# Immortalqx/pi-slam-fusion

Measured on AMD Instinct MI355X. Metric: keyframes/sec fused (4000x3000 -> 256^2 tiles, 5-band), higher is better.
Workload: dtype f32; 1 GPU; cfg-2/cfg-A: 4000x3000 BGR8 keyframes, serpentine sortie, Map2D.Scale=1, 5-band Laplacian, CV_32FC3 (ForceFloat=1) pyramids, frames resident in HBM; frames_per_rank=2646, sortie_frames_before_timing=20, lookahead=48, rendered_rank0=2666, culled_tiles_rank0=490117

## Files before the change

include/pifusion.h:

```cpp
#ifndef PIFUSION_H
#define PIFUSION_H
#include <stddef.h>
#include <stdint.h>

#ifdef __cplusplus
extern "C" {
#endif

#define PF_ELE_PIXELS 256

enum { PF_TYPE_NONE = 0, PF_TYPE_CPU = 1, PF_TYPE_GPU = 2, PF_TYPE_MULTIBAND = 3, PF_TYPE_RENDER = 4 };

enum { PF_8UC1 = 0, PF_8UC3 = 16, PF_8UC4 = 24, PF_16SC3 = 19, PF_32FC1 = 5, PF_32FC3 = 21 };

typedef struct pf_image {
    int         rows, cols, type;
    const void* data;
    size_t      step;
} pf_image;

typedef struct pf_options {
    int    band_number;
    int    force_float;
    int    high_quality_show;
// ... 109 lines not shown
    unsigned long long strips_sent, strips_received, tiles, peers;
    double plan_ms, pack_ms, exchange_ms, compute_ms;
    unsigned long long verified;
} pf_dist_stats;
int      pf_dist_last_stats(pf_dist* d, pf_dist_stats* out);
typedef struct pf_strip_plan { int peer, ix, iy, dx, dy, tile; unsigned long long offset; } pf_strip_plan;
int      pf_dist_plan_blend(int nranks, int me, const int* counts, const int* lists3, const long long* caps, int high_quality,
                            const size_t halo_bytes9[9], pf_strip_plan* send, int send_cap, int* n_send,
                            pf_strip_plan* recv, int recv_cap, int* n_recv, int* mine_xy, int mine_cap, int* n_mine);
int      pf_dist_info(pf_dist* d, int* rank, int* nranks, const char** transport);
int      pf_dist_set_verify(pf_dist* d, int on);

int     pf_profile_enable(pf_map* m, int mode);
int     pf_profile_read(pf_map* m, int cap, const char** names, double* total_ms, long long* launches,
                        double* alg_bytes);
int     pf_profile_read_run(pf_map* m, int cap, const char** names, double* total_ms, long long* launches,
                            double* alg_bytes, double* alg_bytes_run);
int     pf_profile_reset(pf_map* m);
int     pf_render_stats(pf_map* m, double out4[4]);
int     pf_timer_read(pf_map* m, int cap, const char** names, long long* calls, double* mean_s, double* min_s, double* max_s);
int     pf_timer_reset(pf_map* m);
long long pf_debug_culled_tiles(pf_map* m);
long long pf_debug_culled_cells(pf_map* m);
double  pf_debug_level0_exact_px(pf_map* m);
int     pf_debug_render_log(pf_map* m, long long* out, int cap);
void    pf_set_cull(pf_map* m, int on);
void    pf_debug_form_counts(long long out[8]);
long long pf_debug_compact_launches(void);
int     pf_stats(pf_map* m, long long* rendered, long long* rejected, long long* dropped);
int     pf_reserve_tiles(pf_map* m, long long n_tiles);

#ifdef __cplusplus
}
#endif
#endif
```

pi-slam-fusion_amd/__init__.py:

```python
import ctypes as C
import os
import subprocess

import numpy as np

_HERE = os.path.dirname(os.path.abspath(__file__))
LIB_PATH = os.environ.get("PF_LIB") or os.path.join(_HERE, "libpifusion.so")
ELE_PIXELS = 256

NoType, TypeCPU, TypeGPU, TypeMultiBandCPU, TypeRender = 0, 1, 2, 3, 4
PF_8UC3, PF_8UC4, PF_16SC3, PF_32FC3 = 16, 24, 19, 21


def host_array(shape, dtype=np.uint8):
    n = int(np.prod(shape)) * np.dtype(dtype).itemsize
    p = lib().pf_host_alloc(n)
    if not p:
        raise MemoryError("pf_host_alloc(%d)" % n)
    buf = (C.c_uint8 * n).from_address(p)
    a = np.frombuffer(buf, dtype=dtype).reshape(shape)
    import weakref
    weakref.finalize(buf, lib().pf_host_free, p)
    return a

# ... 116 lines not shown
    L.pf_dist_feed.argtypes = [vp, C.POINTER(Image), dp, C.c_int]
    L.pf_dist_feed_jpeg.argtypes = [vp, C.c_char_p, C.c_size_t, C.c_int, C.c_int, dp, C.c_int]
    L.pf_dist_save.argtypes = [vp, C.c_char_p]
    L.pf_dist_save_to_memory.argtypes = [vp, vp, ip, ip, ip, ip]
    L.pf_dist_last_stats.argtypes = [vp, C.POINTER(DistStats)]
    L.pf_dist_info.argtypes = [vp, ip, ip, C.POINTER(C.c_char_p)]
    L.pf_dist_set_verify.argtypes = [vp, C.c_int]
    L.pf_dist_plan_blend.argtypes = [C.c_int, C.c_int, ip, ip, C.POINTER(C.c_longlong), C.c_int, C.POINTER(C.c_size_t), vp, C.c_int, ip,
                                     vp, C.c_int, ip, ip, C.c_int, ip]
    if hasattr(L, "pf_debug_compact_launches") or not os.environ.get("PF_LIB"):
        L.pf_debug_compact_launches.argtypes = []; L.pf_debug_compact_launches.restype = C.c_longlong
    L.pf_profile_enable.argtypes = [vp, C.c_int]
    L.pf_profile_read.argtypes = [vp, C.c_int, C.POINTER(C.c_char_p), dp, C.POINTER(C.c_longlong), dp]
    if hasattr(L, "pf_profile_read_run") or not os.environ.get("PF_LIB"):
        L.pf_profile_read_run.argtypes = [vp, C.c_int, C.POINTER(C.c_char_p), dp, C.POINTER(C.c_longlong), dp, dp]
    L.pf_profile_reset.argtypes = [vp]
    L.pf_stats.argtypes = [vp, C.POINTER(C.c_longlong), C.POINTER(C.c_longlong), C.POINTER(C.c_longlong)]
    L.pf_reserve_tiles.argtypes = [vp, C.c_longlong]
    L.pf_debug_culled_tiles.argtypes = [vp]; L.pf_debug_culled_tiles.restype = C.c_longlong
    L.pf_set_cull.argtypes = [vp, C.c_int]; L.pf_set_cull.restype = None
    if hasattr(L, "pf_debug_render_log") or not os.environ.get("PF_LIB"):
        L.pf_debug_render_log.argtypes = [vp, C.POINTER(C.c_longlong), C.c_int]
    L.pf_debug_culled_cells.argtypes = [vp]; L.pf_debug_culled_cells.restype = C.c_longlong
    L.pf_debug_level0_exact_px.argtypes = [vp]; L.pf_debug_level0_exact_px.restype = C.c_double
    L.pf_render_stats.argtypes = [vp, dp]
    L.pf_timer_read.argtypes = [vp, C.c_int, C.POINTER(C.c_char_p), C.POINTER(C.c_longlong), dp, dp, dp]
    L.pf_timer_reset.argtypes = [vp]
    _lib = L
    return L


POSE7 = C.c_double * 7


def _pose(p):
    if isinstance(p, POSE7):
        return p, p
    a = np.ascontiguousarray(p, dtype=np.float64).reshape(-1)
    return a, a.ctypes.data_as(C.POINTER(C.c_double))


def default_options(**kw):
    o = Options()
    lib().pf_default_options(C.byref(o))
    for k, v in kw.items():
        if not hasattr(o, k):
# ... 432 lines not shown
        cap = 16
        names = (C.c_char_p * cap)(); calls = (C.c_longlong * cap)(); mean = (C.c_double * cap)(); mn = (C.c_double * cap)(); mx = (C.c_double * cap)()
        k = lib().pf_timer_read(self._h, cap, names, calls, mean, mn, mx)
        return {names[i].decode(): {"calls": calls[i], "mean_s": mean[i], "min_s": mn[i], "max_s": mx[i]} for i in range(k)}

    def timer_reset(self):
        lib().pf_timer_reset(self._h)

    def set_cull(self, on):
        lib().pf_set_cull(self._h, 1 if on else 0)

    def render_log(self):
        n = lib().pf_debug_render_log(self._h, None, 0)
        out = (C.c_longlong * max(n, 1))()
        k = lib().pf_debug_render_log(self._h, out, n)
        return [int(out[i]) for i in range(min(n, k))]

    def culled_tiles(self):
        return int(lib().pf_debug_culled_tiles(self._h))

    def culled_cells(self):
        return int(lib().pf_debug_culled_cells(self._h))

    def stats(self):
        a, b, c = C.c_longlong(), C.c_longlong(), C.c_longlong()
        lib().pf_stats(self._h, C.byref(a), C.byref(b), C.byref(c))
        return {"rendered": a.value, "rejected": b.value, "dropped": c.value}
```

pi-slam-fusion_amd/csrc/c_api.cpp:

```cpp
#include "dist.hpp"
#include "jpeg_device.hpp"
#include <cstdlib>
#include <cmath>
#include <cstdio>
#include <cstring>
#include <algorithm>
#include <vector>
#include <mutex>
#include <new>

using pf::FusionMap;

struct pf_map {
    FusionMap impl;
    pf::JpegDevice jpeg;
    pf_map(int t, bool th, const pf_options& o) : impl(t, th, o) {}
    ~pf_map() { if (impl.ok() && impl.use_device()) impl.sync(); }
};

static std::mutex g_jpeg_mu;
static pf::JpegDevice* shared_jpeg(int device = 0)
{
    static pf::JpegDevice* d[64] = {};
    if (device < 0 || device >= 64) device = 0;
// ... 36 lines not shown
{
    if (type == PF_TYPE_NONE || type == PF_TYPE_RENDER) return nullptr;
    pf_options o;
    if (opt) o = *opt; else pf_default_options(&o);
    pf_map* m = new (std::nothrow) pf_map(type, thread != 0, o);
    if (m && !m->impl.ok()) { delete m; return nullptr; }
    return m;
}

void pf_destroy(pf_map* m) { delete m; }
const char* pf_last_error(void) { return pf::last_error(); }

int pf_prepare(pf_map* m, const double plane[7], const double cam[6], int n, const pf_image* imgs, const double* poses7)
{ return m && m->impl.prepare(plane, cam, n, imgs, poses7); }

int pf_feed(pf_map* m, const pf_image* img, const double pose[7]) { return m && m->impl.feed(img, pose, false); }
int pf_feed_device(pf_map* m, const pf_image* img, const double pose[7]) { return m && m->impl.feed(img, pose, true); }
int pf_debug_phase_stamps(unsigned long long* out, int cap_blocks) { return pf::read_phase_stamps(out, cap_blocks); }
void pf_debug_form_counts(long long out[8]) { if (out) pf::read_form_counts(out); }
long long pf_debug_compact_launches(void) { return pf::read_compact_launches(); }
int pf_debug_render_log(pf_map* m, long long* out, int cap) { return m ? m->impl.render_log(out, cap) : 0; }
void pf_set_cull(pf_map* m, int on) { if (m) m->impl.set_cull(on != 0); }
long long pf_debug_culled_cells(pf_map* m) { return m ? m->impl.culled_cells() : 0; }
double pf_debug_level0_exact_px(pf_map* m) { return m ? m->impl.level0_exact_px() : 0; }
long long pf_debug_culled_tiles(pf_map* m) { return m ? m->impl.culled_tiles() : 0; }
int pf_debug_select_counts(unsigned long long* out, int reset) { return out ? pf::read_select_counts(out, reset) : 0; }
long pf_debug_read_last_frame(pf_map* m, void* out, size_t cap) { return m ? m->impl.read_back_last_frame(out, cap) : -1; }
unsigned pf_queue_size(pf_map* m) { return m ? m->impl.queue_size() : 0; }
int pf_sync(pf_map* m) { return m && m->impl.sync(); }
int pf_save(pf_map* m, const char* filename) { return m && filename && m->impl.save(filename); }
int pf_save_tiff(pf_map* m, const char* filename, int quality, int force_bigtiff) { return m && filename && m->impl.save_tiff(filename, quality, force_bigtiff != 0); }
int pf_save_tiff_masked(pf_map* m, const char* filename, int quality, int force_bigtiff) { return m && filename && m->impl.save_tiff_masked(filename, quality, force_bigtiff != 0); }
int pf_jpeg_info(const uint8_t* data, size_t len, int* rows, int* cols, int* components) { return pf::jpeg_info(data, len, rows, cols, components); }
int pf_jpeg_decode_bgr(const uint8_t* data, size_t len, uint8_t* bgr, int rows, int cols)
{ return rows > 0 && cols > 0 && pf::jpeg_decode_bgr(data, len, bgr, rows, cols, (size_t)cols * 3); }
int pf_jpeg_decode_device(const uint8_t* data, size_t len, void* dev_bgr, int rows, int cols, void* hip_stream)
{
    std::lock_guard<std::mutex> l(g_jpeg_mu);
    if (rows <= 0 || cols <= 0 || !dev_bgr) return 0;
    hipPointerAttribute_t at{};
    if (hipPointerGetAttributes(&at, dev_bgr) != hipSuccess || at.type != hipMemoryTypeDevice) { (void)hipGetLastError(); pf::set_error("pf_jpeg_decode_device: destination is not device memory"); return 0; }
    int prev = 0;
    (void)hipGetDevice(&prev);
    if (at.device != prev && hipSetDevice(at.device) != hipSuccess) { pf::set_error("pf_jpeg_decode_device: hipSetDevice failed"); return 0; }
    const int ok = shared_jpeg(at.device)->decode_to(data, len, (uint8_t*)dev_bgr, rows, cols, hip_stream);
    if (at.device != prev) (void)hipSetDevice(prev);
// ... 341 lines not shown
```

pi-slam-fusion_amd/csrc/frame_plan.hpp:

```cpp
#pragma once
#include "plan_limits.hpp"
#include <algorithm>
#include <cmath>
#include <cstdint>
#include <cstring>
#include <vector>

namespace pf {

struct Win { int x0, x1, y0, y1; };


struct CullMargins { double px = 2.0, w = 1e-5; int sub = 4; };

inline bool cull_frame_ok(const double M[9], int crows, int ccols)
{
    const double xs[2] = { -600.0, ccols + 600.0 }, ys[2] = { -600.0, crows + 600.0 };
    int sign = 0;
    for (int i = 0; i < 4; i++) {
        const double x = xs[i & 1], y = ys[i >> 1], W = M[6] * x + M[7] * y + M[8];
        if (!(std::fabs(W) > 1e-12) || !std::isfinite(W)) return false;
        const int sg = W > 0 ? 1 : -1;
        if (sign && sg != sign) return false;
        sign = sg;
// ... 1 lines not shown
    }
    return true;
}

inline float stored_bound(float wlb, bool single_band)
{
    const float gap = single_band ? 3.2f / 254.f : 0.f, floor_w = single_band ? 6.f / 254.f : 0.f;
    return wlb > floor_w ? wlb - gap : 0.f;
}

struct TileCull {
    unsigned out;
    int nraise; int q[16]; float w[16];
};

struct Lattice {
    bool all = false; int nx = 0, ny = 0, dil = 1, cols = 0, rows = 0; double xc = 0, yc = 0, dis_max = 1, inv_dis_max = 1, M[9] = {};
    CullMargins mg;
    std::vector<double> sx, sy, d; std::vector<unsigned char> in;
    std::vector<double> pair_d; std::vector<unsigned char> pair_in; bool paired = false;

    void map_canvas(const double Minv[9], int crows, int ccols, int cols_, int rows_, int dil_, bool map_all, const CullMargins& m)
    {
        all = map_all; mg = m; paired = false;
        dil = dil_;
        nx = ccols / 64 + 2 * dil + 1; ny = crows / 64 + 2 * dil + 1;
        const size_t n = (size_t)nx * ny;
        sx.resize(n); sy.resize(n); d.resize(n); in.assign(n, 2);
        xc = (double)(cols_ / 2); yc = (double)(rows_ / 2); dis_max = std::sqrt(xc * xc + yc * yc);
        inv_dis_max = 1.0 / dis_max;
        cols = cols_; rows = rows_;
        for (int i = 0; i < 9; i++) M[i] = Minv[i];
        if (!map_all) return;
        const double cmax = cols - 2.0, rmax = rows - 2.0;
        for (int m_ = 0; m_ < ny; m_++) {
            const double y = 64.0 * (m_ - dil), n0 = M[1] * y + M[2], n1 = M[4] * y + M[5], w0 = M[7] * y + M[8];
            double* __restrict__ psx = sx.data() + (size_t)m_ * nx; double* __restrict__ psy = sy.data() + (size_t)m_ * nx;
            double* __restrict__ pd = d.data() + (size_t)m_ * nx; unsigned char* __restrict__ pin = in.data() + (size_t)m_ * nx;
            for (int k = 0; k < nx; k++) {
                const double x = 64.0 * (k - dil), iw = 1.0 / (M[6] * x + w0);
                const double px = (M[0] * x + n0) * iw, py = (M[3] * x + n1) * iw, dx = px - xc, dy = py - yc;
                psx[k] = px; psy[k] = py; pd[k] = dx * dx + dy * dy;
            }
            for (int k = 0; k < nx; k++) pin[k] = (unsigned char)((psx[k] >= 1.0) & (psx[k] <= cmax) & (psy[k] >= 1.0) & (psy[k] <= rmax));
        }
    }

// ... 31 lines not shown
        }
        if (!want_out || !(wlb > 2e-5f)) return false;
        double g = (double)wlb - mw;
        if (weight_type != 0) g = std::sqrt(g);
        const double T = mpx + dis_max * (1.0 - g), T2 = T * T;
        if (d2[0] <= T2 || d2[1] <= T2 || d2[2] <= T2 || d2[3] <= T2) return false;
        bool pos = true, neg = true; double dnear2 = 1e300;
        for (int i = 0; i < 4; i++) {
            const size_t a = c[i], b = c[(i + 1) & 3];
            const double ex = sx[b] - sx[a], ey = sy[b] - sy[a], px = xc - sx[a], py = yc - sy[a];
            const double cr = ex * py - ey * px;
            pos = pos && cr >= 0; neg = neg && cr <= 0;
            const double e2 = ex * ex + ey * ey, dot = px * ex + py * ey;
            if (dot > 0 && dot < e2) dnear2 = std::min(dnear2, cr * cr / e2);
        }
        if (pos || neg) return false;
        return dnear2 > T2;
    }

    void raise_bounds(int x, int y, int weight_type, float wlb[16])
    {
        if (all && mg.sub == 4) raise_bounds_fast(x, y, weight_type, wlb); else raise_bounds_cells(x, y, weight_type, wlb);
    }
    void raise_bounds_cells(int x, int y, int weight_type, float wlb[16])
    {
        const int S = mg.sub, span = 4 / S;
        for (int q = 0; q < S * S; q++) {
            float wmin;
            (void)cell_out(4 * x + span * (q % S), 4 * y + span * (q / S), span, weight_type, wlb[q], false, &wmin);
            if (wmin > 0.f && wmin > wlb[q]) wlb[q] = wmin;
        }
    }
    void raise_bounds_fast(int x, int y, int weight_type, float wlb[16])
    {
        const int e = 1 + 2 * dil;
        if (!paired) {
            pair_d.resize((size_t)nx * ny); pair_in.resize((size_t)nx * ny);
            for (int m = 0; m < ny; m++) {
                const double* __restrict__ dd = d.data() + (size_t)m * nx; const unsigned char* __restrict__ ii = in.data() + (size_t)m * nx;
                double* __restrict__ pd = pair_d.data() + (size_t)m * nx; unsigned char* __restrict__ pi = pair_in.data() + (size_t)m * nx;
                for (int k = 0; k + e < nx; k++) { pd[k] = std::max(dd[k], dd[k + e]); pi[k] = ii[k] & ii[k + e]; }
            }
            paired = true;
        }
        const double mpx = mg.px, mw = mg.w;
        for (int qy = 0; qy < 4; qy++) {
// ... 14 lines not shown
    }

    void tile_cull(int x, int y, const float wlb[16], bool fresh, bool lookahead, bool pre_raised, int weight_type, bool single_band, TileCull& c)
    {
        const int S = mg.sub, span = 4 / S;
        c.out = 0; c.nraise = 0;
        bool tile_out = false;
        const bool ask = !fresh || lookahead;
        if (ask) {
            float wl = wlb[0];
            for (int q = 1; q < S * S; q++) wl = std::min(wl, wlb[q]);
            tile_out = cell_out(4 * x, 4 * y, 4, weight_type, stored_bound(wl, single_band), true, nullptr);
        }
        if (tile_out && pre_raised) c.out = 0xffffu;
        else for (int q = 0; q < S * S; q++) {
            const int qx = q % S, qy = q / S;
            float wmin = 0.f;
            if (cell_out(4 * x + span * qx, 4 * y + span * qy, span, weight_type, stored_bound(wlb[q], single_band), ask && !tile_out, pre_raised ? nullptr : &wmin) || tile_out)
                c.out |= S == 4 ? 1u << q : 0x33u << (8 * qy + 2 * qx);
            if (wmin > wlb[q]) { c.q[c.nraise] = q; c.w[c.nraise++] = wmin; }
        }
        if (fresh && c.out != 0xffffu) c.out = 0;
    }
};

inline void clampw(int lo, int hi, int n, int& o0, int& o1) { o0 = std::max(lo, 0); o1 = std::min(hi, n); }
inline int lv_lo(int p, int i) { return p >> i; }
inline int lv_hi(int p, int i) { return (p + (1 << i) - 1) >> i; }

inline void need_windows(const Win& box, int L, int crows, int ccols, Win N[kMaxLevels])
{
    for (int i = L; i >= 0; i--) {
        int x0 = lv_lo(box.x0, i), x1 = lv_hi(box.x1, i), y0 = lv_lo(box.y0, i), y1 = lv_hi(box.y1, i);
        if (i > 0) { x0 -= 1; x1 += 1; y0 -= 1; y1 += 1; }
        if (i < L) {
            x0 = std::min(x0, 2 * N[i + 1].x0 - 2); x1 = std::max(x1, 2 * N[i + 1].x1 + 1);
            y0 = std::min(y0, 2 * N[i + 1].y0 - 2); y1 = std::max(y1, 2 * N[i + 1].y1 + 1);
        }
        clampw(x0, x1, ccols >> i, N[i].x0, N[i].x1);
        clampw(y0, y1, crows >> i, N[i].y0, N[i].y1);
    }
}

typedef unsigned __int128 u128;
inline u128 col_mask(int x0, int x1) { return (x1 - x0 >= 127 ? ~(u128)0 : (((u128)1 << (x1 - x0 + 1)) - 1)) << x0; }

// ... 185 lines not shown
```

pi-slam-fusion_amd/csrc/fusion_map.cpp:

```cpp
#include "fusion_map.hpp"
#include "env.hpp"
#include "warp_index.hpp"
#include "coverage.hpp"
#include <algorithm>
#include <cmath>
#include <cstdio>
#include <cstdlib>
#include <cstring>
#include <chrono>
#include <dlfcn.h>

namespace pf {

static thread_local std::string g_err;
void set_error(const std::string& msg) { g_err = msg; std::fprintf(stderr, "pifusion: %s\n", msg.c_str()); }
const char* last_error() { return g_err.c_str(); }

#define HIP_OK(expr)                                                                       \
    do {                                                                                   \
        hipError_t e_ = (expr);                                                            \
        if (e_ != hipSuccess) {                                                            \
            set_error(std::string(#expr) + ": " + hipGetErrorString(e_));                  \
            return false;                                                                  \
        }                                                                                  \
// ... 330 lines not shown
    std::printf("Map2D.Resolution=%g\n", length_pixel);
    mn[0] = mn[0] - radius; mn[1] = mn[1] - radius;
    mx[0] = mx[0] + radius; mx[1] = mx[1] + radius;
    double ctr[3];
    for (int k = 0; k < 3; k++) ctr[k] = 0.5 * (mn[k] + mx[k]);
    for (int k = 0; k < 3; k++) { mn[k] = 2 * mn[k] - ctr[k]; mx[k] = 2 * mx[k] - ctr[k]; }
    const double ele_size = kElePixels * length_pixel;
    const int w = (int)std::ceil((mx[0] - mn[0]) / ele_size);
    const int h = (int)std::ceil((mx[1] - mn[1]) / ele_size);
    mx[0] = mn[0] + ele_size * w;
    mx[1] = mn[1] + ele_size * h;

    {
        std::unique_lock<std::mutex> q(qmu_);
        for (auto& f : queue_) if (f.slot >= 0) slots_[f.slot].queued = false;
        queue_.clear();
        idle_cv_.wait(q, [this] { return !worker_busy_; });
    }
    std::lock_guard<std::mutex> l(mu_);
    if (!set_device()) return false;
    if (valid_) (void)drain();
    for (auto& p : pending_) release_slot(p.f);
    pending_.clear();
    HIP_OK(sync_all());
    store_.clear();
    plane_ = plane; plane_inv_ = pinv; cam_ = c;
    length_pixel_ = length_pixel; length_pixel_inv_ = 1. / length_pixel;
    ele_size_ = ele_size; ele_size_inv_ = 1. / ele_size;
    std::memcpy(min_, mn, sizeof(mn)); std::memcpy(max_, mx, sizeof(mx));
    w_ = w; h_ = h; off_x_ = off_y_ = 0;
    valid_ = true;
    if (thread_ && imgs) {
        for (int i = 0; i < n; i++) {
            if (!imgs[i].data) continue;
            const int cn = imgs[i].type == PF_8UC4 ? 4 : 3;
            const size_t row_bytes = (size_t)imgs[i].cols * cn, step = imgs[i].step ? imgs[i].step : row_bytes;
            if (step < row_bytes || step * (size_t)imgs[i].rows >= (1ull << 31)) { set_error("prepare: bad row step or frame of 2 GiB or more"); return false; }
            const int slot = acquire_slot((size_t)imgs[i].rows * step);
            if (slot < 0 || !upload(&imgs[i], slot)) return false;
            std::lock_guard<std::mutex> q(qmu_);
            slots_[slot].queued = true;
            queue_.push_back({ slot, nullptr, (long)step, imgs[i].rows, imgs[i].cols, cn, local[i] });
        }
        qcv_.notify_all();
    }
    return true;
// ... 252 lines not shown
    Section sec(this, T_SPREAD);
    Win r;
    tile_range(xmin, ymin, xmax, ymax, r);
    const int xminInt = std::min(r.x0, 0), yminInt = std::min(r.y0, 0);
    const int xmaxInt = std::max(r.x1, w_), ymaxInt = std::max(r.y1, h_);
    const int w = xmaxInt - xminInt, h = ymaxInt - yminInt;
    const double mnx = min_[0] + ele_size_ * xminInt, mny = min_[1] + ele_size_ * yminInt;
    const double mxx = mnx + w * ele_size_, mxy = mny + h * ele_size_;
    min_[0] = mnx; min_[1] = mny; max_[0] = mxx; max_[1] = mxy;
    w_ = w; h_ = h; off_x_ += xminInt; off_y_ += yminInt;
    return true;
}

bool FusionMap::render_frame(const QueuedFrame& f)
{
    Section sec(this, T_RENDER);
    FrameWork& w = fw_;
    w.reset();
    const int go = frame_canvas(f, w);
    if (go <= 0) { release_slot(f); if (go < 0) n_rejected_++; return go == 0; }
    pending_.emplace_back();
    PendingFrame& p = pending_.back();
    p.f = f;
    std::memcpy(p.pts, w.pts, sizeof(p.pts));
    p.sx0 = w.xminInt + off_x_; p.sy0 = w.yminInt + off_y_; p.tx = w.tx; p.ty = w.ty;
    std::memcpy(p.M0, w.M0, sizeof(p.M0));
    w.cull = cull_on_ && (single_band_ || (opt_.fused == 1 && w.L >= 1)) && invert3x3(w.M0, w.Minv) && cull_frame_ok(w.Minv, w.crows, w.ccols);
    p.cull = w.cull;
    std::memcpy(p.Minv, w.Minv, sizeof(p.Minv));
    if (f.slot >= 0) { std::lock_guard<std::mutex> q(qmu_); slots_[f.slot].queued = true; }
    size_t keep = 0;
    if (w.cull) {
        if (!lat_pool_.empty()) { p.lat = std::move(lat_pool_.back()); lat_pool_.pop_back(); }
        w.lat = &p.lat;
        bool map_all = opt_.shard_count <= 1;
        if (!map_all) {
            int mine = 0;
            for (int y = 0; y < w.ty; y++)
                for (int x = 0; x < w.tx; x++) mine += tile_owner(opt_.shard_count, opt_.shard_block, w.xminInt + x + off_x_, w.yminInt + y + off_y_) == opt_.shard_rank;
            map_all = 4 * mine >= w.tx * w.ty;
        }
        p.lat.map_canvas(w.Minv, w.crows, w.ccols, f.cols, f.rows, single_band_ ? 0 : ((2 << w.L) - 2 + 63) / 64, map_all, cull_margins_);
        if (lookahead_ok()) {
            if (!tiles_pool_.empty()) { p.tiles = std::move(tiles_pool_.back()); tiles_pool_.pop_back(); }
            pre_raise(w, p.tiles);
            p.pre_raised = true;
            since_drain_++;
            keep = std::min<size_t>((size_t)opt_.lookahead, 2 * (size_t)since_drain_ / 3);
        }
    }
    while (pending_.size() > keep)
        if (!render_front()) return false;
    return true;
}

void FusionMap::pre_raise(FrameWork& w, std::vector<Tile*>& tiles)
{
    tiles.assign((size_t)w.tx * w.ty, nullptr);
    const bool sharded = opt_.shard_count > 1;
    for (int y = 0; y < w.ty; y++)
        for (int x = 0; x < w.tx; x++) {
            const int sx = w.xminInt + x + off_x_, sy = w.yminInt + y + off_y_;
            if (sharded && tile_owner(opt_.shard_count, opt_.shard_block, sx, sy) != opt_.shard_rank) continue;
            Tile* t = store_.get_or_create(sx, sy);
            if (!t) { tiles.clear(); return; }
            tiles[(size_t)y * w.tx + x] = t;
            w.lat->raise_bounds(x, y, opt_.weight_type, t->wlb);
        }
}

void FusionMap::release_slot(const QueuedFrame& f)
{
    if (f.slot < 0) return;
    std::lock_guard<std::mutex> q(qmu_);
    slots_[f.slot].queued = false;
}

bool FusionMap::drain()
{
    since_drain_ = 0;
    if (pending_.empty()) return true;
    if (!set_device()) return false;
    while (!pending_.empty())
        if (!render_front()) return false;
    return true;
}

bool FusionMap::render_front()
{
    struct Pop {
        FusionMap* m;
        ~Pop() {
            PendingFrame& p = m->pending_.front();
            if (p.lat.sx.capacity() && m->lat_pool_.size() < 8) m->lat_pool_.push_back(std::move(p.lat));
            if (p.tiles.capacity() && m->tiles_pool_.size() < 8) m->tiles_pool_.push_back(std::move(p.tiles));
            m->pending_.pop_front();
        }
    } pop{ this };
    PendingFrame& p = pending_.front();
    const QueuedFrame f = p.f;
    struct Held { FusionMap* m; const QueuedFrame& f; bool done = false; ~Held() { if (!done) m->release_slot(f); } } held{ this, f };
    FrameWork& w = fw_;
    w.reset();
    std::memcpy(w.pts, p.pts, sizeof(p.pts));
    w.xminInt = p.sx0 - off_x_; w.yminInt = p.sy0 - off_y_; w.xmaxInt = w.xminInt + p.tx; w.ymaxInt = w.yminInt + p.ty;
    w.tx = p.tx; w.ty = p.ty; w.L = band_num_; w.crows = w.ty * kElePixels; w.ccols = w.tx * kElePixels;
    std::memcpy(w.M0, p.M0, sizeof(p.M0)); std::memcpy(w.Minv, p.Minv, sizeof(p.Minv));
    w.cull = p.cull;
    w.pre_raised = p.pre_raised;
    w.tiles_known = p.tiles.size() == (size_t)p.tx * p.ty ? p.tiles.data() : nullptr;
    w.src = f.ext ? f.ext : slots_[f.slot].dev;
    w.lat = &p.lat;
    Section sec_apply(this, T_APPLY);
    if (!build_tile_table(f, w)) return false;
    if (w.bx0 >= w.bx1) {
        for (auto& r : w.raise) r.t->wlb[r.q] = std::max(r.t->wlb[r.q], r.w);
        for (Tile* t : w.culled) t->changed = true;
        if (w.owned_all) n_rendered_++;
        log_rendered(f);
        return true;
    }
    px_owned_ += (double)w.owned * kElePixels * kElePixels;
    n_with_pixels_++;
    w.plan.windows(w.pb, w.L, w.crows, w.ccols);
    if (!reserve_frame_workspace(w) || !place_table(w)) return false;
    warp_args(f, w);
    const bool fused = opt_.fused != 0 && w.L >= 1;
    bool ok;
    if (single_band_) ok = launch_single_band(f, w);
    else if (fused) {
        if (wmap_rows_ != f.rows || wmap_cols_ != f.cols) {
            HIP_OK(sync_all());
            if (!wmap_.reserve((size_t)f.rows * f.cols * 4)) return false;
            launch_weight32(stream_, (float*)wmap_.p, f.rows, f.cols, opt_.weight_type);
            wmap_rows_ = f.rows; wmap_cols_ = f.cols;
        }
        w.a.wmap = (const float*)wmap_.p;
        plan_fused_levels(w);
        ok = opt_.fused == 1 ? launch_fused_pipeline(f, w) : launch_level_streams(f, w);
// ... 24 lines not shown
    }
    const double xmin = min_[0] + ele_size_ * w.xminInt, ymin = min_[1] + ele_size_ * w.yminInt;
    w.src = f.ext ? f.ext : (f.slot >= 0 ? slots_[f.slot].dev : nullptr);
    if (!w.src) return 0;
    const float src4[8] = { 0.f, 0.f, (float)cam_.w, 0.f, 0.f, (float)cam_.h, (float)cam_.w, (float)cam_.h };
    float dst4[8];
    for (int i = 0; i < 4; i++) {
        dst4[2 * i]     = (float)((pts[2 * i] - xmin) * length_pixel_inv_);
        dst4[2 * i + 1] = (float)((pts[2 * i + 1] - ymin) * length_pixel_inv_);
    }
    perspective_transform(src4, dst4, w.M0);
    w.tx = w.xmaxInt - w.xminInt; w.ty = w.ymaxInt - w.yminInt; w.L = band_num_;
    w.crows = w.ty * kElePixels; w.ccols = w.tx * kElePixels;
    return 1;
}

bool FusionMap::build_tile_table(const QueuedFrame& f, FrameWork& w)
{
    const int tx = w.tx, ty = w.ty;
    w.sharded = opt_.shard_count > 1;
    const bool sharded = w.sharded;
    const bool cull = w.cull;
    const bool lookahead = cull && lookahead_ok();
    if (cull) w.raise.reserve((size_t)tx * ty * cull_margins_.sub * cull_margins_.sub);
    const int B = opt_.shard_block;
    static const int bc_env = exp_env_int("PF_CULL_CELL", 0);
    const int Bc = sharded ? B : (bc_env > 0 ? bc_env : 8);
    table_tmp_.resize((size_t)tx * ty);
    w.touched.reserve((size_t)tx * ty);
    w.bx0 = tx; w.bx1 = 0; w.by0 = ty; w.by1 = 0;
    w.pb = Win{ 1 << 30, 0, 1 << 30, 0 };
    auto add_rect = [&](int sx, int sy, int x0, int y0, int x1, int y1) {
        w.pb.x0 = std::min(w.pb.x0, x0); w.pb.x1 = std::max(w.pb.x1, x1); w.pb.y0 = std::min(w.pb.y0, y0); w.pb.y1 = std::max(w.pb.y1, y1);
        if (sharded || cull) w.cells.add(floordiv(sx, Bc), floordiv(sy, Bc), x0, y0, x1, y1);
    };
    for (int y = 0; y < ty; y++) {
        const int sy = w.yminInt + y + off_y_;
        for (int x = 0; x < tx; x++) {
            const int sx = w.xminInt + x + off_x_;
            uint64_t ent = 0;
            Tile* known = w.tiles_known ? w.tiles_known[(size_t)y * tx + x] : nullptr;
            if (known || ((!sharded || tile_owner(opt_.shard_count, B, sx, sy) == opt_.shard_rank) && !w.tiles_known)) {
                Tile* t = known ? known : store_.get_or_create(sx, sy);
                if (!t) return false;
                w.owned_all++;
                unsigned out = 0;
                if (cull) {
                    TileCull c;
                    w.lat->tile_cull(x, y, t->wlb, t->fresh, lookahead, w.pre_raised, opt_.weight_type, single_band_, c);
                    out = c.out;
                    for (int k = 0; k < c.nraise; k++) w.raise.push_back(FrameWork::Raise{ t, c.q[k], c.w[k] });
                    if (out == 0xffffu && t->fresh) {
                        w.culled_any = true; table_tmp_[(size_t)y * tx + x] = 0; n_culled_tiles_++;
                        continue;
                    }
                    if (out == 0xffffu) {
                        w.culled_any = true; table_tmp_[(size_t)y * tx + x] = 0; n_culled_tiles_++; w.culled.push_back(t);
                        continue;
                    }
                    if (out) { w.culled_any = true; n_culled_cells_ += __builtin_popcount(out); }
                }
                if ((uint64_t)(uintptr_t)t->base >> 48) { set_error("tile slot address above 2^48: the table entry has no room for the cell flags"); return false; }
                ent = (uint64_t)(uintptr_t)t->base | (t->fresh ? 1u : 0u) | ((uint64_t)out << 48);
                w.touched.push_back(t);
                w.owned++;
                w.bx0 = std::min(w.bx0, x); w.bx1 = std::max(w.bx1, x + 1); w.by0 = std::min(w.by0, y); w.by1 = std::max(w.by1, y + 1);
                if (!out) add_rect(sx, sy, x * kElePixels, y * kElePixels, (x + 1) * kElePixels, (y + 1) * kElePixels);
                else
                    for (int r = 0; r < 4; r++) {
                        const unsigned in = ~(out >> (4 * r)) & 15u;
                        if (!in) continue;
                        const int c0 = __builtin_ctz(in), c1 = 32 - __builtin_clz(in);
                        add_rect(sx, sy, x * kElePixels + 64 * c0, y * kElePixels + 64 * r, x * kElePixels + 64 * c1, y * kElePixels + 64 * r + 64);
// ... 190 lines not shown
        const double ts = kElePixels >> i, n = (double)(w.bx1 - w.bx0) * (w.by1 - w.by0) * ts * ts;
        prof_begin(K_LAP_SELECT, n * (3 * es + 4 + 4) + (i < L ? n / 4 * 3 * es : 0));
        launch_lap_select(stream_, lay_, i, g_[i].p, i < L ? g_[i + 1].p : nullptr, (const float*)wgt_[i].p,
                          w.crows >> i, w.ccols >> i, w.dtab, w.tx, w.by0, w.by1, w.bx0, w.bx1);
        prof_end();
    }
    return true;
}

bool FusionMap::retire_frame(const QueuedFrame& f, FrameWork& w, bool fused)
{
    if (!table_pending_[w.ring] && !(fused && opt_.fused == 1)) {
        if (!submitted()) return false;
        table_release_[w.ring] = work_no_;
    }
    if (f.slot >= 0) {
        const hipError_t e = hipEventRecord(slots_[f.slot].consumed, stream_);
        slots_[f.slot].pending = e == hipSuccess;
        release_slot(f);
        HIP_OK(e);
    }
    for (Tile* t : w.touched) { t->fresh = false; t->changed = true; }
    for (Tile* t : w.culled) t->changed = true;
    for (auto& r : w.raise) r.t->wlb[r.q] = std::max(r.t->wlb[r.q], r.w);
    n_rendered_++;
    log_rendered(f);
    return true;
}

#if PF_EXPERIMENTS
void FusionMap::cull_exact_stat(const FrameWork& w)
{
    const int L = w.L, tx = w.tx, crows = w.crows, ccols = w.ccols, BHr = level_block_rows(lay_.f32 != 0);
    const Win* C = w.plan.C; const LevelPlan& pl = w.plan;
    const int R0 = 94, nbx = (C[0].x1 - C[0].x0 + 63) / 64, nby = (C[0].y1 - C[0].y0 + BHr - 1) / BHr;
    long cnt = 0;
    for (int gy = 0; gy < nby; gy++)
        for (int gx = 0; gx < nbx; gx++) {
            const int x0 = C[0].x0 + gx * 64 - R0, x1 = C[0].x0 + gx * 64 + 63 + R0, y0 = C[0].y0 + gy * BHr - R0, y1 = C[0].y0 + gy * BHr + BHr - 1 + R0;
            bool need = false;
            for (int qy = std::max(y0, 0) >> 6; qy <= (std::min(y1, crows - 1) >> 6) && !need; qy++)
                for (int qx = std::max(x0, 0) >> 6; qx <= (std::min(x1, ccols - 1) >> 6) && !need; qx++) {
                    const uint64_t e = table_tmp_[(size_t)(qy >> 2) * tx + (qx >> 2)];
                    need = e != 0 && !((e >> (48 + (qy & 3) * 4 + (qx & 3))) & 1);
                }
            cnt += need;
        }
// ... 196 lines not shown
}

bool FusionMap::tile_export(int ix, int iy, void* dev_out)
{
    std::lock_guard<std::mutex> l(mu_); (void)drain();
    if (!init_ok_ || !set_device()) return false;
    Tile* t = store_.find(ix, iy);
    if (!t || t->fresh) return false;
    HIP_OK(hipMemcpyAsync(dev_out, t->base, lay_.slot_bytes, hipMemcpyDeviceToDevice, stream_));
    HIP_OK(sync_all());
    return true;
}

bool FusionMap::tile_import(int ix, int iy, const void* dev_in)
{
    std::lock_guard<std::mutex> l(mu_); (void)drain();
    if (!init_ok_ || !valid_ || !set_device()) return false;
    Tile* t = store_.get_or_create(ix, iy);
    if (!t) return false;
    HIP_OK(hipMemcpyAsync(t->base, dev_in, lay_.slot_bytes, hipMemcpyDeviceToDevice, stream_));
    HIP_OK(sync_all());
    t->fresh = false; t->changed = true;
    for (float& w : t->wlb) w = -1.f;
    return true;
}

void FusionMap::list_tiles(std::vector<TileRec>& out)
{
    std::lock_guard<std::mutex> l(mu_); (void)drain();
    out.clear();
    store_.for_each([&](int ix, int iy, Tile& t) { if (!t.fresh) out.push_back({ ix, iy, t.changed ? 1 : 0 }); });
    std::sort(out.begin(), out.end(), [](const TileRec& a, const TileRec& b) { return a.iy != b.iy ? a.iy < b.iy : a.ix < b.ix; });
}

bool FusionMap::pack_strips(const std::vector<StripReq>& reqs, void* dev_out)
{
    std::lock_guard<std::mutex> l(mu_); (void)drain();
    if (!init_ok_ || !set_device()) return false;
    if (reqs.empty()) return true;
    if (!settle()) return false;
    std::vector<StripDesc> d(reqs.size());
    for (size_t i = 0; i < reqs.size(); i++) {
        Tile* t = store_.find(reqs[i].ix, reqs[i].iy);
        if (!t || t->fresh) { set_error("pack_strips: tile not held by this rank"); return false; }
        d[i] = { t->base, reqs[i].dx, reqs[i].dy, reqs[i].out_off };
    }
// ... 546 lines not shown
```

pi-slam-fusion_amd/csrc/fusion_map.hpp:

```cpp
#pragma once
#include "../../include/pifusion.h"
#include "geometry.hpp"
#include "kernels.hpp"
#include "dist_plan.hpp"
#include "frame_plan.hpp"
#include "env.hpp"
#include "image_io.hpp"
#include "jpeg_encode.hpp"
#include "tiff_pyramid.hpp"
#include <hip/hip_runtime.h>
#include <condition_variable>
#include <cstdlib>
#include <deque>
#include <functional>
#include <mutex>
#include <string>
#include <thread>
#include <unordered_map>
#include <vector>

namespace pf {

void set_error(const std::string& msg);
const char* last_error();

int tile_owner(int shard_count, int shard_block, int ix, int iy);

struct Tile {
    char* base = nullptr;
    bool  fresh = true;
    bool  changed = false;
    float wlb[16] = { -1.f, -1.f, -1.f, -1.f, -1.f, -1.f, -1.f, -1.f, -1.f, -1.f, -1.f, -1.f, -1.f, -1.f, -1.f, -1.f };
};

class TileStore {
public:
    ~TileStore() { clear(); }
    void  configure(size_t slot_bytes) { slot_bytes_ = slot_bytes; }
    Tile* find(int ix, int iy);
    Tile* get_or_create(int ix, int iy);
    bool  reserve(size_t n_tiles, std::vector<std::pair<char*, size_t>>* fresh = nullptr);
    void  clear();
    size_t size() const { return map_.size(); }
    template <class F> void for_each(F f) { for (auto& kv : map_) f((int)(int32_t)(kv.first >> 32), (int)(int32_t)(kv.first & 0xffffffffu), kv.second); }
private:
    static uint64_t key(int ix, int iy) { return ((uint64_t)(uint32_t)ix << 32) | (uint32_t)iy; }
    std::unordered_map<uint64_t, Tile> map_;
    struct Chunk { char* p; size_t slots; };
    std::vector<Chunk> chunks_;
    size_t slot_bytes_ = 0, cur_ = 0, next_in_chunk_ = 0;
    bool   add_chunk(size_t slots);
};

struct DevBuf {
    void*  p = nullptr;
// ... 62 lines not shown
    bool save_to_memory(uint8_t* bgr, int* rows, int* cols, int* tx0, int* ty0) { return save_to_memory_mask(bgr, nullptr, rows, cols, tx0, ty0); }
    bool save_to_memory_mask(uint8_t* bgr, uint8_t* mask, int* rows, int* cols, int* tx0, int* ty0);
    bool save_to_memory_level(int level, uint8_t* bgr, int* rows, int* cols, int* tx0, int* ty0);

    using TileRec = pf::TileRec;
    using StripReq = pf::StripReq;
    void list_tiles(std::vector<TileRec>& out);
    bool pack_strips(const std::vector<StripReq>& reqs, void* dev_out);
    bool export_tiles(const std::vector<std::pair<int, int>>& tiles, void* dev_out);
    bool blend_tiles(const std::vector<std::pair<int, int>>& tiles, const void* const* halo9, uint8_t* bgr);
    bool reject_mismatched_frame(const pf_image* desc);
    bool frame_needs(const double pose7[7], std::vector<unsigned char>& rank_needs);
    int  stage_frame(const pf_image* desc, bool upload_host, void** dev, size_t* bytes);
    bool feed_staged(int slot, const pf_image* desc, const double pose7[7]);
    void release_staged(int slot) { std::lock_guard<std::mutex> q(qmu_); if (slot >= 0 && slot < (int)slots_.size()) slots_[slot].queued = false; }
    hipStream_t stream() const { return stream_; }
    int  device() const { return device_; }
    bool use_device() { return set_device(); }
    bool single_band() const { return single_band_; }
    bool map_update_inputs(int ix, int iy, double plane7[7], double mn[2], double* ele, int* x, int* y);
    long long culled_tiles() { std::lock_guard<std::mutex> l(mu_); (void)drain(); return n_culled_tiles_; }
    void set_cull(bool on) { std::lock_guard<std::mutex> l(mu_); (void)drain(); cull_on_ = on; }
    long long culled_cells() { std::lock_guard<std::mutex> l(mu_); (void)drain(); return n_culled_cells_; }
    int  render_log(long long* out, int cap);
    double level0_exact_px() const { return px_level0_exact_; }
    bool high_quality() const { return opt_.high_quality_show != 0 && !single_band_; }

    int  num_levels() const { return band_num_ + 1; }
    int  pyramid_type() const { return single_band_ ? PF_8UC4 : (lay_.f32 ? PF_32FC3 : PF_16SC3); }
    bool grid(int dims[4], double geo[6]);
    int  tile_count();
    int  tile_coords(int* xy, int cap);
    bool get_tile_level(int ix, int iy, int level, void* lap, float* w);
    bool get_tile_bgra(int ix, int iy, uint8_t* bgra);
    bool blend_tile(int ix, int iy, void* raw, uint8_t* bgr, const void* const* halo);
    int  blend_changed(int* xy, uint8_t* bgr, int cap, int level = 0);
    bool blend_list(const std::vector<std::pair<int, int>>& tiles, uint8_t* bgr);
    bool blend_list_level(const std::vector<std::pair<int, int>>& tiles, int level, uint8_t* bgr, void* raw);
    bool level_ok(const char* who, int level);
    struct TileJpeg { int quality; uint8_t* out; size_t cap; size_t* offsets; size_t used = 0; };
    bool blend_list_jpeg(const std::vector<std::pair<int, int>>& tiles, int quality, uint8_t* out, size_t cap, size_t* offsets);
    size_t halo_bytes_for(int dx, int dy) const { return halo_bytes(lay_, dx, dy); }
    bool halo_pack(int ix, int iy, int dx, int dy, void* dev_out);
    size_t tile_bytes() const { return lay_.slot_bytes; }
    bool tile_export(int ix, int iy, void* dev_out);
    bool tile_import(int ix, int iy, const void* dev_in);
// ... 26 lines not shown
    void prof_begin(int id, double bytes, hipStream_t st = nullptr, double bytes_run = -1);
    bool prof_would(int id) const;
    hipError_t sync_all();
    void prof_end();
    void prof_harvest();
    bool set_device();

    pf_options opt_;
    int        band_num_ = 5;
    TileLayout lay_{};
    bool       thread_ = false, init_ok_ = false;
    bool       single_band_ = false;
    DevBuf     w8_; int w8_rows_ = 0, w8_cols_ = 0;
    DevBuf     wmap_; int wmap_rows_ = 0, wmap_cols_ = 0;
    int        device_ = 0;
    hipStream_t stream_ = nullptr;

    std::mutex mu_;
    bool   valid_ = false;
    Pose   plane_{}, plane_inv_{};
    bool cull_on_ = !(std::getenv("PF_CULL") && std::atoi(std::getenv("PF_CULL")) == 0);
    long long n_culled_tiles_ = 0;
    long long n_culled_cells_ = 0;
    CullMargins cull_margins_{ exp_env_double("PF_CULL_MARGIN_PX", 2.0), exp_env_double("PF_CULL_MARGIN_W", 1e-5), exp_env_int("PF_CULL_SUB", 4) == 2 ? 2 : 4 };
    Camera cam_{};
    double ele_size_ = 0, ele_size_inv_ = 0, length_pixel_ = 0, length_pixel_inv_ = 0;
    double min_[3]{}, max_[3]{};
    int    w_ = 0, h_ = 0, off_x_ = 0, off_y_ = 0;
    TileStore store_;

    DevBuf g_[kMaxLevels], wgt_[kMaxLevels], gw_[kMaxLevels], gw2_[kMaxLevels];
    hipStream_t lvl_stream_[kMaxLevels]{};
    static constexpr int kTableRing = 64;
    static constexpr int kLvlRing = 16;
    hipEvent_t  lvl_ev_[kMaxLevels][kLvlRing]{};
    hipStream_t prof_stream_ = nullptr;
    static constexpr int kUpperStreams = 1;
    uint64_t*  table_host_[kTableRing]{};
    bool       table_in_args_ = true;
    DevBuf     table_dev_[kTableRing];
    std::vector<uint64_t> table_tmp_;
    size_t     table_cap_ = 0;
    hipEvent_t table_ev_[kTableRing]{};
    bool       table_pending_[kTableRing]{};
    static constexpr int kMarkEvery = 32, kMarks = 4;
    unsigned long long work_no_ = 0, synced_no_ = 0;
    unsigned long long table_release_[kTableRing]{};
    hipEvent_t mark_ev_[kMarks]{};
    unsigned long long mark_no_[kMarks]{};
    int  mark_next_ = 0;
    bool submitted();
    bool wait_for(unsigned long long no);
    unsigned long long frame_seq_ = 0;

    struct PipeFrame { bool valid = false; int ring = 0, tx = 0, crows = 0, ccols = 0; Win C[kMaxLevels]; double bytes[kMaxLevels], bytes_run[kMaxLevels];
                       int nrect[kMaxLevels]; BlockRect rect[kMaxLevels][kMaxRects];
                       uint32_t need_bits[kMaxLevels][kNeedWords]; int need_n[kMaxLevels] = {};
                       const uint64_t* table_args = nullptr; int table_n = 0; };
    PipeFrame pipe_[kMaxLevels];
    struct FrameWork {
        double pts[8]; int xminInt, yminInt, xmaxInt, ymaxInt;
        int tx, ty, L, crows, ccols; double M0[9], Minv[9];
        const uint8_t* src;
        bool sharded, cull, culled_any; Lattice* lat;
        bool pre_raised;
        Tile* const* tiles_known;
        struct Raise { Tile* t; int q; float w; };
        std::vector<Raise> raise; std::vector<Tile*> culled, touched;
        CellList cells;
        int bx0, bx1, by0, by1, owned, owned_all;
        Win pb;
        LevelPlan plan;
        int ring; bool table_args; const uint64_t* dtab;
        WarpArgs a;
        void reset() {
            raise.clear(); culled.clear(); touched.clear();
            culled_any = cells.overflow = false; cells.n = 0; owned = owned_all = 0; plan.reset();
            src = nullptr; ring = 0; table_args = false; dtab = nullptr; sharded = cull = pre_raised = false; tiles_known = nullptr; lat = nullptr;
        }
    };
    FrameWork fw_;
    struct PendingFrame {
        QueuedFrame f;
        double pts[8]; int sx0, sy0, tx, ty;
        double M0[9], Minv[9];
        bool cull;
        Lattice lat;
        bool pre_raised = false;
        std::vector<Tile*> tiles;
    };
    std::deque<PendingFrame> pending_;
    unsigned since_drain_ = 0;
    std::vector<Lattice> lat_pool_;
    std::vector<std::vector<Tile*>> tiles_pool_;
    bool lookahead_ok() const { return opt_.lookahead > 0 && (single_band_ || (opt_.fused == 1 && band_num_ >= 1)) && cull_on_; }
    bool render_front();
    bool drain();
    void release_slot(const QueuedFrame& f);
    void pre_raise(FrameWork& w, std::vector<Tile*>& tiles);
    int  frame_canvas(const QueuedFrame& f, FrameWork& w);
    bool build_tile_table(const QueuedFrame& f, FrameWork& w);
    bool reserve_frame_workspace(FrameWork& w);
    bool place_table(FrameWork& w);
    void warp_args(const QueuedFrame& f, FrameWork& w);
    void plan_fused_levels(FrameWork& w);
    bool launch_single_band(const QueuedFrame& f, FrameWork& w);
    bool launch_fused_pipeline(const QueuedFrame& f, FrameWork& w);
    bool launch_level_streams(const QueuedFrame& f, FrameWork& w);
    bool launch_per_op(const QueuedFrame& f, FrameWork& w);
    bool retire_frame(const QueuedFrame& f, FrameWork& w, bool fused);
    void log_rendered(const QueuedFrame& f);
    unsigned long long launch_seq_ = 0;
    bool flushing_ = false;
    bool launch_pipeline(const PipeFrame* cur, const WarpArgs* wa, const uint8_t* src);
    bool flush_pipeline();
    bool settle();
// ... 47 lines not shown
```

Baseline: 28220 keyframes/s.

## Cull cells using pairwise lattice comparison against the frame that set the weight bound

Records, per tile sub-cell, which keyframe last raised its weight lower bound, and keeps recent frame lattices in a ring. During tile culling, a non-fresh cell can now be skipped when a geometric pairwise test shows the current frame's weight upper bound is below the recording frame's lower bound over the cell neighbourhood. This is meant to reject more cells from GPU blending work, at the cost of extra host CPU work per tile and memory for kept lattices, and it adds some correctness risk if the bounds are not conservative.

Result: slower. 18080 keyframes/s (-35.9%).

```diff
diff --git a/include/pifusion.h b/include/pifusion.h
--- a/include/pifusion.h
+++ b/include/pifusion.h
@@ -155,6 +155,7 @@
 int     pf_timer_reset(pf_map* m);
 long long pf_debug_culled_tiles(pf_map* m);
 long long pf_debug_culled_cells(pf_map* m);
+long long pf_debug_pair_culled_cells(pf_map* m);
 double  pf_debug_level0_exact_px(pf_map* m);
 int     pf_debug_render_log(pf_map* m, long long* out, int cap);
 void    pf_set_cull(pf_map* m, int on);
diff --git a/pi-slam-fusion_amd/__init__.py b/pi-slam-fusion_amd/__init__.py
--- a/pi-slam-fusion_amd/__init__.py
+++ b/pi-slam-fusion_amd/__init__.py
@@ -162,6 +162,8 @@
     if hasattr(L, "pf_debug_render_log") or not os.environ.get("PF_LIB"):
         L.pf_debug_render_log.argtypes = [vp, C.POINTER(C.c_longlong), C.c_int]
     L.pf_debug_culled_cells.argtypes = [vp]; L.pf_debug_culled_cells.restype = C.c_longlong
+    if hasattr(L, "pf_debug_pair_culled_cells") or not os.environ.get("PF_LIB"):
+        L.pf_debug_pair_culled_cells.argtypes = [vp]; L.pf_debug_pair_culled_cells.restype = C.c_longlong
     L.pf_debug_level0_exact_px.argtypes = [vp]; L.pf_debug_level0_exact_px.restype = C.c_double
     L.pf_render_stats.argtypes = [vp, dp]
     L.pf_timer_read.argtypes = [vp, C.c_int, C.POINTER(C.c_char_p), C.POINTER(C.c_longlong), dp, dp, dp]
@@ -640,6 +642,9 @@
     def culled_cells(self):
         return int(lib().pf_debug_culled_cells(self._h))
 
+    def pair_culled_cells(self):
+        return int(lib().pf_debug_pair_culled_cells(self._h))
+
     def stats(self):
         a, b, c = C.c_longlong(), C.c_longlong(), C.c_longlong()
         lib().pf_stats(self._h, C.byref(a), C.byref(b), C.byref(c))
diff --git a/pi-slam-fusion_amd/csrc/c_api.cpp b/pi-slam-fusion_amd/csrc/c_api.cpp
--- a/pi-slam-fusion_amd/csrc/c_api.cpp
+++ b/pi-slam-fusion_amd/csrc/c_api.cpp
@@ -82,6 +82,7 @@
 int pf_debug_render_log(pf_map* m, long long* out, int cap) { return m ? m->impl.render_log(out, cap) : 0; }
 void pf_set_cull(pf_map* m, int on) { if (m) m->impl.set_cull(on != 0); }
 long long pf_debug_culled_cells(pf_map* m) { return m ? m->impl.culled_cells() : 0; }
+long long pf_debug_pair_culled_cells(pf_map* m) { return m ? m->impl.pair_culled_cells() : 0; }
 double pf_debug_level0_exact_px(pf_map* m) { return m ? m->impl.level0_exact_px() : 0; }
 long long pf_debug_culled_tiles(pf_map* m) { return m ? m->impl.culled_tiles() : 0; }
 int pf_debug_select_counts(unsigned long long* out, int reset) { return out ? pf::read_select_counts(out, reset) : 0; }
diff --git a/pi-slam-fusion_amd/csrc/frame_plan.hpp b/pi-slam-fusion_amd/csrc/frame_plan.hpp
--- a/pi-slam-fusion_amd/csrc/frame_plan.hpp
+++ b/pi-slam-fusion_amd/csrc/frame_plan.hpp
@@ -47,7 +47,7 @@
 
     void map_canvas(const double Minv[9], int crows, int ccols, int cols_, int rows_, int dil_, bool map_all, const CullMargins& m)
     {
-        all = map_all; mg = m; paired = false;
+        all = map_all; mg = m; paired = false; squared = false;
         dil = dil_;
         nx = ccols / 64 + 2 * dil + 1; ny = crows / 64 + 2 * dil + 1;
         const size_t n = (size_t)nx * ny;
@@ -125,6 +125,13 @@
     {
         if (all && mg.sub == 4) raise_bounds_fast(x, y, weight_type, wlb); else raise_bounds_cells(x, y, weight_type, wlb);
     }
+    void raise_bounds(int x, int y, int weight_type, float wlb[16], uint32_t by[16], uint32_t serial)
+    {
+        float before[16];
+        std::memcpy(before, wlb, sizeof(before));
+        raise_bounds(x, y, weight_type, wlb);
+        for (int q = 0; q < 16; q++) if (wlb[q] != before[q]) by[q] = serial;
+    }
     void raise_bounds_cells(int x, int y, int weight_type, float wlb[16])
     {
         const int S = mg.sub, span = 4 / S;
@@ -185,6 +192,78 @@
         }
         if (fresh && c.out != 0xffffu) c.out = 0;
     }
+
+    void squares_ready()
+    {
+        if (squared) return;
+        sq_near.assign((size_t)nx * ny, -1.0); sq_far.assign((size_t)nx * ny, -2.0);
+        squared = true;
+    }
+    double square_ub(int k, int m)
+    {
+        squares_ready();
+        double& v = sq_near[(size_t)m * nx + k];
+        if (v >= 0) return v;
+        const size_t c[4] = { point(k, m), point(k + 1, m), point(k + 1, m + 1), point(k, m + 1) };
+        bool pos = true, neg = true;
+        double dn2 = std::min(std::min(d[c[0]], d[c[1]]), std::min(d[c[2]], d[c[3]]));
+        for (int i = 0; i < 4; i++) {
+            const size_t a = c[i], b = c[(i + 1) & 3];
+            const double ex = sx[b] - sx[a], ey = sy[b] - sy[a], px = xc - sx[a], py = yc - sy[a];
+            const double cr = ex * py - ey * px;
+            pos = pos && cr >= 0; neg = neg && cr <= 0;
+            const double e2 = ex * ex + ey * ey, dot = px * ex + py * ey;
+            if (dot > 0 && dot < e2) dn2 = std::min(dn2, cr * cr / e2);
+        }
+        v = (pos || neg) ? 0.0 : std::sqrt(dn2);
+        return v;
+    }
+    double square_lb(int k, int m)
+    {
+        squares_ready();
+        double& v = sq_far[(size_t)m * nx + k];
+        if (v >= -1.0) return v;
+        const size_t c[4] = { point(k, m), point(k + 1, m), point(k + 1, m + 1), point(k, m + 1) };
+        v = (in[c[0]] & in[c[1]] & in[c[2]] & in[c[3]]) == 1 ? std::sqrt(std::max(std::max(d[c[0]], d[c[1]]), std::max(d[c[2]], d[c[3]]))) : -1.0;
+        return v;
+    }
+    double weight_at(double dist, int weight_type) const
+    {
+        const double t = 1.0 - dist * inv_dis_max;
+        return weight_type == 0 ? t : (t > 0 ? t * t : 0.0);
+    }
+    bool pair_out(int kx, int ky, int span, int weight_type, Lattice& g, int dx, int dy)
+    {
+        const int e = span + 2 * dil, gx = kx + dx, gy = ky + dy;
+        if (&g == this || g.dil != dil) return false;
+        if (kx < dil || ky < dil || kx + e > nx - 1 - dil || ky + e > ny - 1 - dil) return false;
+        if (gx < g.dil || gy < g.dil || gx + e > g.nx - 1 - g.dil || gy + e > g.ny - 1 - g.dil) return false;
+        if (e * e > kMaxSquares) return false;
+        double lbs[kMaxSquares];
+        for (int j = 0; j < e; j++)
+            for (int i = 0; i < e; i++) {
+                const double far = g.square_lb(gx + i, gy + j);
+                if (far < 0) return false;
+                const double lb = g.weight_at(far + g.mg.px, weight_type) - g.mg.w;
+                if (!(lb > 2e-5)) return false;
+                double v = lb - mg.w;
+                if (!(v > 0)) return false;
+                if (weight_type != 0) v = std::sqrt(v);
+                const double T = mg.px + dis_max * (1.0 - v), T2 = T * T;
+                const size_t o = (size_t)(ky + j) * nx + kx + i;
+                (void)point(kx + i, ky + j); (void)point(kx + i + 1, ky + j); (void)point(kx + i, ky + j + 1); (void)point(kx + i + 1, ky + j + 1);
+                if (d[o] <= T2 || d[o + 1] <= T2 || d[o + nx] <= T2 || d[o + nx + 1] <= T2) return false;
+                lbs[j * e + i] = lb;
+            }
+        for (int j = 0; j < e; j++)
+            for (int i = 0; i < e; i++) {
+                const double ub = weight_at(square_ub(kx + i, ky + j) - mg.px, weight_type) + mg.w;
+                if (!(ub < lbs[j * e + i])) return false;
+            }
+        return true;
+    }
+    static constexpr int kMaxSquares = 81;
+    std::vector<double> sq_near, sq_far; bool squared = false;
 };
 
 inline void clampw(int lo, int hi, int n, int& o0, int& o1) { o0 = std::max(lo, 0); o1 = std::min(hi, n); }
diff --git a/pi-slam-fusion_amd/csrc/fusion_map.cpp b/pi-slam-fusion_amd/csrc/fusion_map.cpp
--- a/pi-slam-fusion_amd/csrc/fusion_map.cpp
+++ b/pi-slam-fusion_amd/csrc/fusion_map.cpp
@@ -376,6 +376,8 @@
     if (valid_) (void)drain();
     for (auto& p : pending_) release_slot(p.f);
     pending_.clear();
+    lat_ring_.clear();
+    kf_serial_ = 0;
     HIP_OK(sync_all());
     store_.clear();
     plane_ = plane; plane_inv_ = pinv; cam_ = c;
@@ -674,6 +676,8 @@
     pending_.emplace_back();
     PendingFrame& p = pending_.back();
     p.f = f;
+    p.serial = ++kf_serial_;
+    w.serial = p.serial;
     std::memcpy(p.pts, w.pts, sizeof(p.pts));
     p.sx0 = w.xminInt + off_x_; p.sy0 = w.yminInt + off_y_; p.tx = w.tx; p.ty = w.ty;
     std::memcpy(p.M0, w.M0, sizeof(p.M0));
@@ -717,7 +721,7 @@
             Tile* t = store_.get_or_create(sx, sy);
             if (!t) { tiles.clear(); return; }
             tiles[(size_t)y * w.tx + x] = t;
-            w.lat->raise_bounds(x, y, opt_.weight_type, t->wlb);
+            w.lat->raise_bounds(x, y, opt_.weight_type, t->wlb, t->wlb_by, w.serial);
         }
 }
 
@@ -738,13 +742,33 @@
     return true;
 }
 
+Lattice* FusionMap::lattice_of(uint32_t serial, int* sx0, int* sy0)
+{
+    if (!pending_.empty() && serial >= pending_.front().serial) {
+        const size_t i = serial - pending_.front().serial;
+        if (i >= pending_.size() || !pending_[i].cull || pending_[i].serial != serial) return nullptr;
+        *sx0 = pending_[i].sx0; *sy0 = pending_[i].sy0;
+        return &pending_[i].lat;
+    }
+    if (lat_ring_.empty()) return nullptr;
+    KeptLattice& k = lat_ring_[serial % kLatRing];
+    if (k.serial != serial) return nullptr;
+    *sx0 = k.sx0; *sy0 = k.sy0;
+    return &k.lat;
+}
+
 bool FusionMap::render_front()
 {
     struct Pop {
         FusionMap* m;
         ~Pop() {
             PendingFrame& p = m->pending_.front();
-            if (p.lat.sx.capacity() && m->lat_pool_.size() < 8) m->lat_pool_.push_back(std::move(p.lat));
+            if (p.cull && p.lat.sx.capacity() && !m->single_band_ && m->cull_pair_) {
+                if (m->lat_ring_.empty()) m->lat_ring_.resize(kLatRing);
+                KeptLattice& k = m->lat_ring_[p.serial % kLatRing];
+                if (k.lat.sx.capacity() && m->lat_pool_.size() < 8) m->lat_pool_.push_back(std::move(k.lat));
+                k.serial = p.serial; k.sx0 = p.sx0; k.sy0 = p.sy0; k.lat = std::move(p.lat);
+            } else if (p.lat.sx.capacity() && m->lat_pool_.size() < 8) m->lat_pool_.push_back(std::move(p.lat));
             if (p.tiles.capacity() && m->tiles_pool_.size() < 8) m->tiles_pool_.push_back(std::move(p.tiles));
             m->pending_.pop_front();
         }
@@ -760,13 +784,14 @@
     std::memcpy(w.M0, p.M0, sizeof(p.M0)); std::memcpy(w.Minv, p.Minv, sizeof(p.Minv));
     w.cull = p.cull;
     w.pre_raised = p.pre_raised;
+    w.serial = p.serial; w.sx0 = p.sx0; w.sy0 = p.sy0;
     w.tiles_known = p.tiles.size() == (size_t)p.tx * p.ty ? p.tiles.data() : nullptr;
     w.src = f.ext ? f.ext : slots_[f.slot].dev;
     w.lat = &p.lat;
     Section sec_apply(this, T_APPLY);
     if (!build_tile_table(f, w)) return false;
     if (w.bx0 >= w.bx1) {
-        for (auto& r : w.raise) r.t->wlb[r.q] = std::max(r.t->wlb[r.q], r.w);
+        w.apply_raise();
         for (Tile* t : w.culled) t->changed = true;
         if (w.owned_all) n_rendered_++;
         log_rendered(f);
@@ -837,6 +862,8 @@
     const bool sharded = w.sharded;
     const bool cull = w.cull;
     const bool lookahead = cull && lookahead_ok();
+    const bool pair = cull && cull_pair_ && !single_band_;
+    uint32_t cand_serial = 0; Lattice* cand = nullptr; int cand_sx0 = 0, cand_sy0 = 0;
     if (cull) w.raise.reserve((size_t)tx * ty * cull_margins_.sub * cull_margins_.sub);
     const int B = opt_.shard_block;
     static const int bc_env = exp_env_int("PF_CULL_CELL", 0);
@@ -864,6 +891,18 @@
                     TileCull c;
                     w.lat->tile_cull(x, y, t->wlb, t->fresh, lookahead, w.pre_raised, opt_.weight_type, single_band_, c);
                     out = c.out;
+                    if (pair && !t->fresh && out != 0xffffu) {
+                        const int S = cull_margins_.sub, span = 4 / S;
+                        for (int q = 0; q < S * S; q++) {
+                            const unsigned bits = S == 4 ? 1u << q : 0x33u << (8 * (q / S) + 2 * (q % S));
+                            const uint32_t by = t->wlb_by[q];
+                            if ((out & bits) || !by || by == w.serial) continue;
+                            if (by != cand_serial) { cand_serial = by; cand = lattice_of(by, &cand_sx0, &cand_sy0); }
+                            if (cand && w.lat->pair_out(4 * x + span * (q % S), 4 * y + span * (q / S), span, opt_.weight_type, *cand, 4 * (w.sx0 - cand_sx0), 4 * (w.sy0 - cand_sy0))) {
+                                out |= bits; n_pair_cells_ += span * span;
+                            }
+                        }
+                    }
                     for (int k = 0; k < c.nraise; k++) w.raise.push_back(FrameWork::Raise{ t, c.q[k], c.w[k] });
                     if (out == 0xffffu && t->fresh) {
                         w.culled_any = true; table_tmp_[(size_t)y * tx + x] = 0; n_culled_tiles_++;
@@ -1100,7 +1139,7 @@
     }
     for (Tile* t : w.touched) { t->fresh = false; t->changed = true; }
     for (Tile* t : w.culled) t->changed = true;
-    for (auto& r : w.raise) r.t->wlb[r.q] = std::max(r.t->wlb[r.q], r.w);
+    w.apply_raise();
     n_rendered_++;
     log_rendered(f);
     return true;
@@ -1343,6 +1382,7 @@
     HIP_OK(sync_all());
     t->fresh = false; t->changed = true;
     for (float& w : t->wlb) w = -1.f;
+    for (uint32_t& b : t->wlb_by) b = 0;
     return true;
 }
 
diff --git a/pi-slam-fusion_amd/csrc/fusion_map.hpp b/pi-slam-fusion_amd/csrc/fusion_map.hpp
--- a/pi-slam-fusion_amd/csrc/fusion_map.hpp
+++ b/pi-slam-fusion_amd/csrc/fusion_map.hpp
@@ -31,6 +31,7 @@
     bool  fresh = true;
     bool  changed = false;
     float wlb[16] = { -1.f, -1.f, -1.f, -1.f, -1.f, -1.f, -1.f, -1.f, -1.f, -1.f, -1.f, -1.f, -1.f, -1.f, -1.f, -1.f };
+    uint32_t wlb_by[16] = {};
 };
 
 class TileStore {
@@ -139,6 +140,7 @@
     long long culled_tiles() { std::lock_guard<std::mutex> l(mu_); (void)drain(); return n_culled_tiles_; }
     void set_cull(bool on) { std::lock_guard<std::mutex> l(mu_); (void)drain(); cull_on_ = on; }
     long long culled_cells() { std::lock_guard<std::mutex> l(mu_); (void)drain(); return n_culled_cells_; }
+    long long pair_culled_cells() { std::lock_guard<std::mutex> l(mu_); (void)drain(); return n_pair_cells_; }
     int  render_log(long long* out, int cap);
     double level0_exact_px() const { return px_level0_exact_; }
     bool high_quality() const { return opt_.high_quality_show != 0 && !single_band_; }
@@ -211,6 +213,8 @@
     bool cull_on_ = !(std::getenv("PF_CULL") && std::atoi(std::getenv("PF_CULL")) == 0);
     long long n_culled_tiles_ = 0;
     long long n_culled_cells_ = 0;
+    long long n_pair_cells_ = 0;
+    bool cull_pair_ = exp_env_int("PF_CULL_PAIR", 1) != 0;
     CullMargins cull_margins_{ exp_env_double("PF_CULL_MARGIN_PX", 2.0), exp_env_double("PF_CULL_MARGIN_W", 1e-5), exp_env_int("PF_CULL_SUB", 4) == 2 ? 2 : 4 };
     Camera cam_{};
     double ele_size_ = 0, ele_size_inv_ = 0, length_pixel_ = 0, length_pixel_inv_ = 0;
@@ -253,8 +257,10 @@
         const uint8_t* src;
         bool sharded, cull, culled_any; Lattice* lat;
         bool pre_raised;
+        uint32_t serial; int sx0, sy0;
         Tile* const* tiles_known;
         struct Raise { Tile* t; int q; float w; };
+        void apply_raise() { for (auto& r : raise) if (r.w > r.t->wlb[r.q]) { r.t->wlb[r.q] = r.w; r.t->wlb_by[r.q] = serial; } }
         std::vector<Raise> raise; std::vector<Tile*> culled, touched;
         CellList cells;
         int bx0, bx1, by0, by1, owned, owned_all;
@@ -266,6 +272,7 @@
             raise.clear(); culled.clear(); touched.clear();
             culled_any = cells.overflow = false; cells.n = 0; owned = owned_all = 0; plan.reset();
             src = nullptr; ring = 0; table_args = false; dtab = nullptr; sharded = cull = pre_raised = false; tiles_known = nullptr; lat = nullptr;
+            serial = 0; sx0 = sy0 = 0;
         }
     };
     FrameWork fw_;
@@ -274,6 +281,7 @@
         double pts[8]; int sx0, sy0, tx, ty;
         double M0[9], Minv[9];
         bool cull;
+        uint32_t serial = 0;
         Lattice lat;
         bool pre_raised = false;
         std::vector<Tile*> tiles;
@@ -281,6 +289,11 @@
     std::deque<PendingFrame> pending_;
     unsigned since_drain_ = 0;
     std::vector<Lattice> lat_pool_;
+    static constexpr uint32_t kLatRing = 128;
+    struct KeptLattice { uint32_t serial = 0; int sx0 = 0, sy0 = 0; Lattice lat; };
+    std::vector<KeptLattice> lat_ring_;
+    uint32_t kf_serial_ = 0;
+    Lattice* lattice_of(uint32_t serial, int* sx0, int* sy0);
     std::vector<std::vector<Tile*>> tiles_pool_;
     bool lookahead_ok() const { return opt_.lookahead > 0 && (single_band_ || (opt_.fused == 1 && band_num_ >= 1)) && cull_on_; }
     bool render_front();
```
